# sidiso/surfh

Hardware: AMD Instinct MI355X
Metric: CG-iterations/sec (forward+adjoint) on 251x251x4000 cube (higher is better)
Workload: dtype f32 (storage and accumulation; products as 2-piece fp16 splits -- 3 products per fp32 product, 1 on the far tails of the spectral response -- on the 16-bit matrix cores, in the spectral-blur GEMM and in the DFT passes)

## Files before the change

surfh_amd/csrc/gemm_cc16.hip:

```cpp
#include "gemm_f32.h"
#include "f16_split.h"
#include "lds_attr.h"
#include <cmath>
#include <cstdlib>
#include <type_traits>

typedef float f32x16 __attribute__((ext_vector_type(16)));
typedef _Float16 f16x8 __attribute__((ext_vector_type(8)));
typedef _Float16 f16x4 __attribute__((ext_vector_type(4)));

namespace {

constexpr int BM = 256, BN = 256, BK = 32;
constexpr int ROWS = BM + BN;
constexpr int PIECE = ROWS * BK;
constexpr int STAGE = 2 * PIECE;
constexpr size_t LDS_BYTES = (size_t)2 * STAGE * sizeof(unsigned short);

__global__ __launch_bounds__(256) void split_rows2h_kernel(const float *__restrict__ src, const unsigned *__restrict__ rowmax,
                                                           unsigned short *__restrict__ dst, int ld, long plane) {
    const int row = blockIdx.y;
    const float inv = 1.f / f16x2_scale(__uint_as_float(rowmax[row]));
    const int k4 = (blockIdx.x * 256 + threadIdx.x) * 4;
    if (k4 >= ld) return;
// ... 38 lines not shown

#define CC_MFMA_DRAIN() asm volatile("s_nop 15\n\ts_nop 15\n\ts_nop 7" ::: "memory")

typedef float f32x4v __attribute__((ext_vector_type(4)));

template <int U, int N, bool DMA, bool FAR>
__device__ __forceinline__ void cc16_slot(f32x4v (&acc)[4][8], f16x8 (&A)[4][2], const f16x8 (&Bc)[2][2], f16x8 (&Bn)[2][2], unsigned ran,
                                          unsigned rbn, const char *ka, const char *kb, long pA2, long pB2, const unsigned (&offA)[2],
                                          const unsigned (&offB)[2], unsigned ls) {
    constexpr int i = N / 6, jj = (N / 3) & 1, j = 2 * U + jj, p = N % 3;
    if constexpr (!(CC_EXP & 4) && (!FAR || p == 2))
        asm volatile("v_mfma_f32_16x16x32_f16 %0, %1, %2, %0" : "+v"(acc[i][j]) : "v"(A[i][p == 0 ? 1 : 0]), "v"(Bc[jj][p == 1 ? 1 : 0]));
    if constexpr (N < 4 && !(CC_EXP & 2)) {
        constexpr int jn = 2 * ((U + 1) & 3) + (N >> 1), q = N & 1;
        if constexpr (!FAR || q == 0)
            asm volatile("ds_read_b128 %0, %1 offset:%2" : "=v"(Bn[N >> 1][q]) : "v"(rbn), "n"(q * PIECE * 2 + jn * 16 * BK * 2));
    }
    if constexpr (U == 3 && N % 6 == 5 && !(CC_EXP & 2)) {
        asm volatile("ds_read_b128 %0, %1 offset:%2" : "=v"(A[i][0]) : "v"(ran), "n"(i * 16 * BK * 2));
        if constexpr (!FAR) asm volatile("ds_read_b128 %0, %1 offset:%2" : "=v"(A[i][1]) : "v"(ran), "n"(PIECE * 2 + i * 16 * BK * 2));
    }
    constexpr int d = (U == 3 && N % 3 != 2 && N < 12) ? N - N / 3 : -1;
    if constexpr (DMA && d >= 0 && !(CC_EXP & 1) && (!FAR || d < 4)) {
        constexpr int q = d >> 2, i2 = (d >> 1) & 1;
        if constexpr (d & 1) cc2_dma(kb + q * pB2, offB[i2], ls + (unsigned)((q * PIECE + (BM + i2 * 128) * BK) * 2));
        else cc2_dma(ka + q * pA2, offA[i2], ls + (unsigned)((q * PIECE + i2 * 128 * BK) * 2));
    }
}
template <int U, bool DMA, bool FAR, int N = 0>
__device__ __forceinline__ void cc16_unit(f32x4v (&acc)[4][8], f16x8 (&A)[4][2], const f16x8 (&Bc)[2][2], f16x8 (&Bn)[2][2], unsigned ran,
                                          unsigned rbn, const char *ka, const char *kb, long pA2, long pB2, const unsigned (&offA)[2],
                                          const unsigned (&offB)[2], unsigned ls) {
    if constexpr (N < 24) {
        if constexpr (U == 0 && N == 18 && !(CC_EXP & 2)) {
            if constexpr (FAR) asm volatile("s_waitcnt lgkmcnt(3)" : "+v"(A[3][0]), "+v"(A[3][1]));
            else asm volatile("s_waitcnt lgkmcnt(5)" : "+v"(A[3][0]), "+v"(A[3][1]));
        }
        cc16_slot<U, N, DMA, FAR>(acc, A, Bc, Bn, ran, rbn, ka, kb, pA2, pB2, offA, offB, ls);
        cc16_unit<U, DMA, FAR, N + 1>(acc, A, Bc, Bn, ran, rbn, ka, kb, pA2, pB2, offA, offB, ls);
    }
}
#define CC16_WAITB(n_, B_)                                                                                              \
    asm volatile("s_waitcnt lgkmcnt(" #n_ ")" : "+v"(B_[0][0]), "+v"(B_[1][0]), "+v"(B_[0][1]), "+v"(B_[1][1]))

constexpr int CC2_MAXLIST = 2048;
constexpr size_t LDS3_BYTES = LDS2_BYTES + (size_t)CC2_MAXLIST * sizeof(int);

struct GemmGroup {
    GemmArgs g[GEMM_GROUP_MAX];
    long first[GEMM_GROUP_MAX + 1];
    int n;
};

__global__ __launch_bounds__(512, 1) void gemm_nt_f16x2_cc_kernel(GemmGroup grp) {
    extern __shared__ __attribute__((aligned(16))) unsigned short lds[];
    const long gtotal = grp.first[grp.n], per = (gtotal + 7) / 8;
    const long vg = (long)(blockIdx.x & 7) * per + (blockIdx.x >> 3);
    if ((long)(blockIdx.x >> 3) >= per || vg >= gtotal) return;
    int gi = 0;
    while (gi + 1 < grp.n && vg >= grp.first[gi + 1]) ++gi;
    const long v = vg - grp.first[gi];
    const GemmArgs g = grp.g[gi];
    unsigned char *sctab = reinterpret_cast<unsigned char *>(lds + 2 * STAGE);
    int *klds = reinterpret_cast<int *>(sctab + CC2_MAXSEG * BM);
    const int tid = threadIdx.x, lane = tid & 63, wave = __builtin_amdgcn_readfirstlane(tid >> 6);
    const int Q = g.permP ? BN / g.permP : BN, tilesL = g.permP ? g.permLin / Q : 0, ncol = g.permP ? g.N / g.permLin : 0;
    const int tilesM = (g.M + BM - 1) / BM, tilesN = g.permP ? (ncol + g.permP - 1) / g.permP * tilesL : (g.N + BN - 1) / BN, tiles = tilesM * tilesN;
    auto bcol = [&](int tn_, int v) __attribute__((always_inline)) {
        if (!g.permP) { const int n = tn_ * BN + v; return n < g.N ? n : -1; }
        const int c = (tn_ / tilesL) * g.permP + v / Q;
        return c < ncol ? c * g.permLin + (tn_ % tilesL) * Q + v % Q : -1;
    };
    const int t = (int)(v % tiles), z = (int)(v / tiles);
    const int tm = t % tilesM, tn = t / tilesM;
    const int b = z / g.splitK, sk = z % g.splitK;
    const int m0 = tm * BM;
    const float *bs = g.bscale;

    int nnear, nfar, seg0 = 0, nseg = 0;
    if (g.klist) {
        const int *kl = g.klist + (long)tn * g.klistStride;
        const int NN = kl[0], NF = kl[1];
        const int a0 = (int)((long)NN * sk / g.splitK), a1 = (int)((long)NN * (sk + 1) / g.splitK);
        const int f0 = (int)((long)NF * sk / g.splitK), f1 = (int)((long)NF * (sk + 1) / g.splitK);
        nnear = __builtin_amdgcn_readfirstlane(a1 - a0);
        nfar = __builtin_amdgcn_readfirstlane(f1 - f0);
        for (int e = tid; e < nnear; e += 512) klds[e] = kl[2 + a0 + e];
        for (int e = tid; e < nfar; e += 512) klds[nnear + e] = kl[2 + NN + f0 + e];
        if (bs) nseg = (g.K / g.segLinP) * g.segChunks;
    } else {
        const int Kper = g.K / g.splitK, kbeg = sk * Kper;
        nnear = Kper / BK;
        nfar = 0;
        if (bs) {
            seg0 = cc2_seg_of(kbeg, g.segLinP, g.segChunks);
            nseg = cc2_seg_of(kbeg + Kper - 1, g.segLinP, g.segChunks) - seg0 + 1;
        }
        for (int e = tid; e < nnear; e += 512) {
            const int k = kbeg + e * BK;
            klds[e] = (k / BK) | (bs ? ((k / g.segLinP) * g.segChunks + (k % g.segLinP) / 1024) << 16 : 0);
        }
    }
    for (int e = tid; e < nseg * BM; e += 512) {
        int row = m0 + (e & (BM - 1));
        row = row < g.M ? row : g.M - 1;
        sctab[e] = (unsigned char)(__float_as_uint(bs[(long)(seg0 + (e >> 8)) * g.M + row]) >> 23);
    }

    unsigned offA[2], offB[2];
    {
        const int chunk = (lane & 3) ^ ((-(lane >> 4)) & 3);
#pragma unroll
        for (int i = 0; i < 2; ++i) {
            int m = m0 + (wave + 8 * i) * 16 + (lane >> 2);
            m = m < g.M ? m : g.M - 1;
            offA[i] = (unsigned)(((long)m * g.lda + 8 * chunk) * 2);
            int n = bcol(tn, (wave + 8 * i) * 16 + (lane >> 2));
            n = n >= 0 ? n : g.N - 1;
            offB[i] = (unsigned)(((long)n * g.ldb + 8 * chunk) * 2);
        }
    }
    const char *baseA = cc2_uniform(reinterpret_cast<const char *>(g.A3 + (long)b * g.sA));
    const char *baseB = cc2_uniform(reinterpret_cast<const char *>(g.B16 + (long)b * g.sB));
    const long pA2 = g.pA3 * 2, pB2 = g.pB16 * 2;
    const unsigned ldsw = (unsigned)(size_t)lds + (unsigned)(wave * 16 * BK * 2);
    const unsigned kaddr = (unsigned)(size_t)klds;
    const int l15 = lane & 15, kc = lane >> 4;
    const int wm = wave >> 1, wn = wave & 1;
    f32x4v acc[4][8];
#pragma unroll
    for (int i = 0; i < 4; ++i)
#pragma unroll
        for (int j = 0; j < 8; ++j) acc[i][j] = f32x4v{0.f, 0.f, 0.f, 0.f};
    const unsigned ra0 = (unsigned)(size_t)lds + (unsigned)(((wm * 64 + l15) * BK + ((kc ^ ((-(l15 >> 2)) & 3)) * 8)) * 2);
    const unsigned fbd = (unsigned)((BM + wn * 128 - wm * 64) * BK * 2);
    const bool active = m0 + wm * 64 < g.M;
    const int srow = wm * 64 + 4 * kc;
    int seg = -1;

    f16x8 A[4][2], Bx[2][2], By[2][2];
#define CC_RD(dst_, addr_, off_) asm volatile("ds_read_b128 %0, %1 offset:%2" : "=v"(dst_) : "v"(addr_), "n"(off_))
#define CC_DMA(FAR_, ks_, st_)                                                                                         \
    {                                                                                                                  \
        const char *ka = baseA + (long)(ks_) * (BK * 2), *kb = baseB + (long)(ks_) * (BK * 2);                         \
        const unsigned ls = ldsw + stofs((FAR_), (st_));                                                               \
        _Pragma("unroll") for (int q = 0; q < ((FAR_) ? 1 : 2); ++q) {                                                 \
            _Pragma("unroll") for (int i = 0; i < 2; ++i) {                                                            \
                cc2_dma(ka + q * pA2, offA[i], ls + (q * PIECE + i * 128 * BK) * 2);                                   \
                cc2_dma(kb + q * pB2, offB[i], ls + (q * PIECE + (BM + i * 128) * BK) * 2);                            \
            }                                                                                                          \
        }                                                                                                              \
    }
    auto stofs = [](bool far, int s) __attribute__((always_inline)) {
        return far ? (unsigned)((s >> 1) * (STAGE * 2) + (s & 1) * (PIECE * 2)) : (unsigned)(s * (STAGE * 2));
    };
    __syncthreads();

    auto kloop = [&](auto far_tag, const int lb, const int n) __attribute__((always_inline)) {
        constexpr bool FAR = decltype(far_tag)::value;
        constexpr int D = FAR ? 4 : 2;
        if (n <= 0) return;
        int e[D];
#pragma unroll
        for (int s = 0; s < D; ++s) {
            e[s] = __builtin_amdgcn_readfirstlane(klds[lb + (s < n ? s : n - 1)]);
            CC_DMA(FAR, e[s] & 0xFFFF, s);
        }
        if (FAR) asm volatile("s_waitcnt vmcnt(12)" ::: "memory");
        else asm volatile("s_waitcnt vmcnt(8)" ::: "memory");
        __syncthreads();
        if (!active) {
            for (int kt = 0; kt < n; ++kt) {
                if (FAR) asm volatile("s_waitcnt vmcnt(8)\n\ts_barrier" ::: "memory");
                else asm volatile("s_waitcnt vmcnt(0)\n\ts_barrier" ::: "memory");
                const int ed = __builtin_amdgcn_readfirstlane(klds[lb + (kt + D < n ? kt + D : n - 1)]);
                CC_DMA(FAR, ed & 0xFFFF, kt & (D - 1));
            }
            asm volatile("s_waitcnt vmcnt(0)" ::: "memory");
            return;
        }
        unsigned ra = ra0, rb = ra0 + fbd;
        if (!(CC_EXP & 2)) {
#pragma unroll
            for (int i = 0; i < 4; ++i) {
                CC_RD(A[i][0], ra, 0 + 0);
                if (!FAR) CC_RD(A[i][1], ra, PIECE * 2);
                ra += 16 * BK * 2;
            }
            ra -= 4 * 16 * BK * 2;
            CC_RD(Bx[0][0], rb, 0); CC_RD(Bx[1][0], rb, 16 * BK * 2);
            if (!FAR) { CC_RD(Bx[0][1], rb, PIECE * 2); CC_RD(Bx[1][1], rb, PIECE * 2 + 16 * BK * 2); }
            asm volatile("s_waitcnt lgkmcnt(0)" : "+v"(A[0][0]), "+v"(A[0][1]), "+v"(A[1][0]), "+v"(A[1][1]), "+v"(A[2][0]), "+v"(A[2][1]), "+v"(A[3][0]),
                         "+v"(A[3][1]), "+v"(Bx[0][0]), "+v"(Bx[1][0]), "+v"(Bx[0][1]), "+v"(Bx[1][1]));
        }
        for (int kt = 0; kt < n; ++kt) {
            const int nseg_ = e[0] >> 16;
            if (bs && nseg_ != seg) {
                if (seg >= 0) {
                    const unsigned char *to = sctab + (seg - seg0) * BM + srow, *tn_ = sctab + (nseg_ - seg0) * BM + srow;
                    unsigned so[4], sn[4];
                    bool same = true;
#pragma unroll
                    for (int i = 0; i < 4; ++i) {
                        so[i] = *reinterpret_cast<const unsigned *>(to + i * 16);
                        sn[i] = *reinterpret_cast<const unsigned *>(tn_ + i * 16);
                        same = same && so[i] == sn[i];
                    }
                    if (__builtin_amdgcn_ballot_w64(!same) != 0ull) {
                        CC_MFMA_DRAIN();
#pragma unroll
                        for (int i = 0; i < 4; ++i) {
                            const f32x4v rt = {cc2_pow2_ratio(so[i] & 255u, sn[i] & 255u), cc2_pow2_ratio((so[i] >> 8) & 255u, (sn[i] >> 8) & 255u),
                                               cc2_pow2_ratio((so[i] >> 16) & 255u, (sn[i] >> 16) & 255u), cc2_pow2_ratio(so[i] >> 24, sn[i] >> 24)};
#pragma unroll
                            for (int j = 0; j < 8; ++j) acc[i][j] *= rt;
                            __builtin_amdgcn_sched_barrier(0);
                        }
                    }
                }
                seg = nseg_;
            }
            unsigned ev;
            asm volatile("ds_read_b32 %0, %1" : "=v"(ev) : "v"(kaddr + 4u * (unsigned)(lb + (kt + D < n ? kt + D : n - 1))));
            const char *kz = baseA;
            const unsigned ls2 = ldsw + stofs(FAR, kt & (D - 1));
            cc16_unit<0, false, FAR>(acc, A, Bx, By, ra, rb, kz, kz, pA2, pB2, offA, offB, ls2);
            asm volatile("s_waitcnt lgkmcnt(0)" : "+v"(By[0][0]), "+v"(By[1][0]), "+v"(By[0][1]), "+v"(By[1][1]), "+v"(ev));
            const int en = __builtin_amdgcn_readfirstlane((int)ev);
            const char *ka2 = baseA + (long)(en & 0xFFFF) * (BK * 2), *kb2 = baseB + (long)(en & 0xFFFF) * (BK * 2);
            cc16_unit<1, false, FAR>(acc, A, By, Bx, ra, rb, kz, kz, pA2, pB2, offA, offB, ls2);
            CC16_WAITB(0, Bx);
            cc16_unit<2, false, FAR>(acc, A, Bx, By, ra, rb, kz, kz, pA2, pB2, offA, offB, ls2);
            CC16_WAITB(0, By);
            if (FAR) asm volatile("s_waitcnt vmcnt(8)\n\ts_barrier" ::: "memory");
            else asm volatile("s_waitcnt vmcnt(0)\n\ts_barrier" ::: "memory");
            {
                const unsigned nx = stofs(FAR, (kt + 1) & (D - 1));
                ra = ra0 + nx; rb = ra0 + fbd + nx;
            }
            cc16_unit<3, true, FAR>(acc, A, By, Bx, ra, rb, ka2, kb2, pA2, pB2, offA, offB, ls2);
            if (FAR) { CC16_WAITB(1, Bx); }
            else { CC16_WAITB(2, Bx); }
#pragma unroll
            for (int s = 0; s + 1 < D; ++s) e[s] = e[s + 1];
            e[D - 1] = en;
        }
        asm volatile("s_waitcnt vmcnt(0) lgkmcnt(0)" ::: "memory");
    };
    kloop(std::false_type{}, 0, nnear);
    if (nfar > 0) {
        __syncthreads();
        kloop(std::true_type{}, nnear, nfar);
    }
    if (!active) return;
    CC_MFMA_DRAIN();
#undef CC_DMA
#undef CC_RD
    {
        char *Cb = reinterpret_cast<char *>(g.C + (long)b * g.sC + (long)sk * g.sCsplit + (long)m0 * g.ldc);
        int cj[8];
#pragma unroll
        for (int j = 0; j < 8; ++j) {
            const int c0 = bcol(tn, wn * 128 + j * 16);
            cj[j] = c0 >= 0 ? c0 + l15 : -1;
        }
        const unsigned ldc4 = (unsigned)(g.ldc * 4);
#pragma unroll
        for (int i = 0; i < 4; ++i) {
            float rsc[4];
#pragma unroll
            for (int r = 0; r < 4; ++r) {
                const int lr = srow + i * 16 + r;
                int row = m0 + lr;
                row = row < g.M ? row : g.M - 1;
                rsc[r] = bs ? (seg >= 0 ? __uint_as_float((unsigned)sctab[(seg - seg0) * BM + lr] << 23) : 1.f) : f16x2_scale(__uint_as_float(g.amax[(long)b * g.M + row]));
            }
#pragma unroll
            for (int r = 0; r < 4; ++r) {
                const int row = m0 + srow + i * 16 + r;
                const float sc = rsc[r] * g.sB16;
                const unsigned o_ = (unsigned)(srow + i * 16 + r) * ldc4;
#pragma unroll
                for (int j = 0; j < 8; ++j)
                    if (row < g.M && cj[j] >= 0 && cj[j] < g.N) *reinterpret_cast<float *>(Cb + (o_ + (unsigned)cj[j] * 4u)) = acc[i][j][r] * sc;
            }
        }
    }
}
#undef CC16_WAITB

__global__ __launch_bounds__(256) void split2h_kernel(const float *__restrict__ src, unsigned short *__restrict__ dst, long n4, long plane,
                                                      float inv) {
    const long stride = (long)gridDim.x * 256;
    for (long i = (long)blockIdx.x * 256 + threadIdx.x; i < n4; i += stride) {
        const float4 v = reinterpret_cast<const float4 *>(src)[i];
        const float x0 = v.x * inv, x1 = v.y * inv, x2 = v.z * inv, x3 = v.w * inv;
        const _Float16 h0 = (_Float16)x0, h1 = (_Float16)x1, h2 = (_Float16)x2, h3 = (_Float16)x3;
        f16x4 h = {h0, h1, h2, h3};
        f16x4 l = {(_Float16)(x0 - (float)h0), (_Float16)(x1 - (float)h1), (_Float16)(x2 - (float)h2), (_Float16)(x3 - (float)h3)};
        *reinterpret_cast<f16x4 *>(dst + 4 * i) = h;
        *reinterpret_cast<f16x4 *>(dst + plane + 4 * i) = l;
    }
}

}

float gemm_f16x2_scale(float amax) {
    if (!(amax > 0.f)) return 1.f;
    int e = 0;
    std::frexp(amax, &e);
    int s = (e - 1) - 13;
    s = s < -126 ? -126 : (s > 127 ? 127 : s);
    return std::ldexp(1.f, s);
}

int launch_split2h(hipStream_t stream, const float *src, unsigned short *dst2, long n, long plane, float scale) {
    if (n % 4 || plane % 4 || !(scale > 0.f)) return (int)hipErrorInvalidValue;
    const long n4 = n / 4;
    long nb = (n4 + 255) / 256;
    hipLaunchKernelGGL(split2h_kernel, dim3((unsigned)(nb > 4096 ? 4096 : (nb < 1 ? 1 : nb))), dim3(256), 0, stream, src, dst2, n4, plane,
                       1.f / scale);
    return (int)hipGetLastError();
}

int launch_split_rows2h(hipStream_t stream, const float *src, const unsigned *rowmax, unsigned short *dst2, int rows, int ld, long plane) {
    if (ld % 4 || plane % 4 || rows < 1) return (int)hipErrorInvalidValue;
    hipLaunchKernelGGL(split_rows2h_kernel, dim3((ld / 4 + 255) / 256, rows), dim3(256), 0, stream, src, rowmax, dst2, ld, plane);
    return (int)hipGetLastError();
}

static int check_gemm_nt_f16x2_cc(const GemmArgs &g, long *items) {
    if (g.M % 64 || g.N % 128 || g.K % (BK * g.splitK) || g.splitK < 1 || g.batch < 1 || g.accumulate || g.lda % 8 || g.ldb % 8 || !g.A3 ||
        !g.B16 || g.pA3 % 8 || g.pB16 % 8 || (!g.amax && !g.bscale) || !(g.sB16 > 0.f))
        return (int)hipErrorInvalidValue;
    if (g.bscale && (g.batch != 1 || g.segLinP < BK || g.segLinP % BK || g.segChunks != (g.segLinP + 1023) / 1024 || g.K % g.segLinP))
        return (int)hipErrorInvalidValue;
    if ((double)(BM + 1) * (double)g.ldc * 4.0 >= 2147483648.0) return (int)hipErrorInvalidValue;
    if ((double)g.M * (double)g.lda * 2.0 >= 4294967296.0 || (double)g.N * (double)g.ldb * 2.0 >= 4294967296.0) return (int)hipErrorInvalidValue;
    if (g.klist) {
        if (g.batch != 1 || g.klistStride < 2 + g.K / BK || g.K / BK > CC2_MAXLIST || g.K / BK > 0xFFFF) return (int)hipErrorInvalidValue;
        if (g.bscale && (g.K / g.segLinP) * g.segChunks > CC2_MAXSEG) return (int)hipErrorInvalidValue;
    } else {
        const int Kper = g.K / g.splitK;
        if (Kper / BK > CC2_MAXLIST || g.K / BK > 0xFFFF) return (int)hipErrorInvalidValue;
        if (g.bscale) {
            auto seg_of = [&](int k) { return (k / g.segLinP) * g.segChunks + (k % g.segLinP) / 1024; };
            for (int sk = 0; sk < g.splitK; ++sk)
                if (seg_of(sk * Kper + Kper - 1) - seg_of(sk * Kper) + 1 > CC2_MAXSEG) return (int)hipErrorInvalidValue;
        }
    }
    long tilesN = (g.N + BN - 1) / BN;
    if (g.permP) {
        if ((g.permP != 1 && g.permP != 2 && g.permP != 4 && g.permP != 8) || g.permLin < 1 || g.permLin % (BN / g.permP) || g.N % g.permLin)
            return (int)hipErrorInvalidValue;
        tilesN = (long)((g.N / g.permLin + g.permP - 1) / g.permP) * (g.permLin / (BN / g.permP));
    }
    *items = (long)((g.M + BM - 1) / BM) * tilesN * g.batch * g.splitK;
    return 0;
}

int launch_gemm_nt_f16x2_cc_group(hipStream_t stream, const GemmArgs *gs, int n) {
    if (n < 1 || n > GEMM_GROUP_MAX) return (int)hipErrorInvalidValue;
    GemmGroup grp;
    grp.n = n;
    grp.first[0] = 0;
    for (int i = 0; i < n; ++i) {
        long items = 0;
        if (int e = check_gemm_nt_f16x2_cc(gs[i], &items)) return e;
        grp.g[i] = gs[i];
        grp.first[i + 1] = grp.first[i] + items;
    }
    for (int i = n; i < GEMM_GROUP_MAX; ++i) grp.first[i + 1] = grp.first[n];
    const long total = grp.first[n];
    if (total >= 2147483647L - 8) return (int)hipErrorInvalidValue;
    dim3 grid((unsigned)(8 * ((total + 7) / 8)));
    static unsigned long long attr_done = 0;
    if (int e = ensure_dynamic_lds(gemm_nt_f16x2_cc_kernel, LDS3_BYTES, attr_done)) return e;
    hipLaunchKernelGGL(gemm_nt_f16x2_cc_kernel, grid, dim3(512), LDS3_BYTES, stream, grp);
    return (int)hipGetLastError();
}

int launch_gemm_nt_f16x2_cc(hipStream_t stream, const GemmArgs &g) { return launch_gemm_nt_f16x2_cc_group(stream, &g, 1); }
```

surfh_amd/csrc/gemm_f32.h:

```cpp
#pragma once
#include <hip/hip_runtime.h>
#include <stdint.h>

struct GemmArgs {
    const float *A0 = nullptr, *A1 = nullptr;
    int ksplitA = 1 << 30;
    long lda = 0, sA = 0;
    const float *B0 = nullptr, *B1 = nullptr;
    int ksplitB = 1 << 30;
    long ldb = 0, sB = 0;
    float *C = nullptr;
    long ldc = 0, sC = 0;
    int M = 0, N = 0, K = 0;
    int batch = 1;
    int splitK = 1;
    long sCsplit = 0;
    int accumulate = 0;
    const unsigned short *A3 = nullptr, *B16 = nullptr;
    long pA3 = 0, pB16 = 0;
    float sB16 = 0.f;
    const unsigned *amax = nullptr;
    const float *bscale = nullptr;
    int segLinP = 0, segChunks = 0;
    const int *klist = nullptr;
    int klistStride = 0;
    int permP = 0, permLin = 0;
};

int launch_gemm_f32(hipStream_t stream, const GemmArgs &g);
int launch_gemm_f64acc(hipStream_t stream, const GemmArgs &g);

int launch_split2h(hipStream_t stream, const float *src, unsigned short *dst2, long n, long plane, float scale);
float gemm_f16x2_scale(float amax);
int launch_gemm_nt_f16x2_cc(hipStream_t stream, const GemmArgs &g);
constexpr int GEMM_GROUP_MAX = 4;
int launch_gemm_nt_f16x2_cc_group(hipStream_t stream, const GemmArgs *g, int n);
int launch_split_rows2h(hipStream_t stream, const float *src, const unsigned *rowmax, unsigned short *dst2, int rows, int ld, long plane);
```

surfh_amd/csrc/plan.hip:

```cpp
#include "plan_internal.h"

#include <atomic>

namespace surfh_impl {

namespace {
thread_local std::string g_err;
}

int fail(const char *fmt, ...) {
    char buf[1024];
    va_list ap;
    va_start(ap, fmt);
    vsnprintf(buf, sizeof buf, fmt, ap);
    va_end(ap);
    g_err = buf;
    return 1;
}

namespace {
std::atomic<int64_t> g_alloc_live{0}, g_alloc_total{0}, g_alloc_fail_at{0};
}
int dev_raw_alloc(void **p, size_t bytes) {
    *p = nullptr;
// ... 655 lines not shown
    const Route r0 = decide_route(rin, OTF_NONE);
    const bool ilv = r0.interleaved();
    {
        const int nkb = p->Nb / 2 + 1;
        const size_t nsp = (size_t)2 * p->PL * LP;
        if (p->sotf.zeros(nsp)) return bail(1);
        std::vector<float> row((size_t)2 * p->KBP * LP);
        for (int a = 0; a < p->Na; ++a) {
            std::fill(row.begin(), row.end(), 0.f);
            for (int l = 0; l < p->Lown; ++l) {
                if (p->planes[l] < 0) continue;
                const double *src = cfg->sotf ? cfg->sotf + ((size_t)p->planes[l] * p->Na + a) * nkb * 2 : nullptr;
                for (int k = 0; k < nkb; ++k) {
                    const float vr = src ? (float)src[2 * k] : 1.f, vi = src ? (float)src[2 * k + 1] : 0.f;
                    if (ilv) {
                        row[((size_t)k * LP + l) * 2] = vr;
                        row[((size_t)k * LP + l) * 2 + 1] = vi;
                    } else {
                        row[(size_t)k * LP + l] = vr;
                        row[((size_t)p->KBP + k) * LP + l] = vi;
                    }
                }
            }
            if (ilv) {
                if (hipMemcpy(p->sotf + (size_t)a * p->KBP * LP * 2, row.data(), (size_t)2 * p->KBP * LP * sizeof(float),
                              hipMemcpyHostToDevice) != hipSuccess)
                    return bail(fail("sotf upload failed"));
            } else
            for (int c = 0; c < 2; ++c)
                if (hipMemcpy(p->sotf + ((size_t)c * p->PL + (size_t)a * p->KBP) * LP, row.data() + (size_t)c * p->KBP * LP,
                              (size_t)p->KBP * LP * sizeof(float), hipMemcpyHostToDevice) != hipSuccess)
                    return bail(fail("sotf upload failed"));
        }
    }
    if (p->T > 0) {
        std::vector<float> t((size_t)p->T * LP, 0.f);
        for (int k = 0; k < p->T; ++k)
            for (int l = 0; l < p->Lown; ++l)
                if (p->planes[l] >= 0) t[(size_t)k * LP + l] = (float)cfg->templates[(size_t)k * p->Lc + p->planes[l]];
        if (p->tpl.upload(t)) return bail(1);
        p->tpl_host.assign(cfg->templates, cfg->templates + (size_t)p->T * p->Lc);
    }
    {
        std::vector<float> Fi, Gi, Gf, Ff, GiT, GfT;
        build_dft(p, Fi, Gi, Gf, Ff, GiT, GfT);
        if (p->Fi.upload(Fi) || p->Gi.upload(Gi) || p->Gf.upload(Gf) || p->Ff.upload(Ff) || p->GiT.upload(GiT) || p->GfT.upload(GfT)) return bail(1);
    }
    {
        p->wblur_fp32 = env_on("SURFH_WBLUR_FP32", false);
        p->overlap = env_on("SURFH_OVERLAP", false);
        if (p->overlap && hipStreamCreateWithFlags(&p->stream2, hipStreamNonBlocking) != hipSuccess) return bail(fail("hipStreamCreate failed"));
        p->gather_grouped = env_on("SURFH_GATHER_GROUPED", true);
        p->gemm_grouped = env_on("SURFH_GEMM_GROUPED", true);
        p->scatter_grouped = env_on("SURFH_SCATTER_GROUPED", true);
        p->gather_sorted = env_on("SURFH_GATHER_SORTED", true);
        const int ha = p->Na / 2 + 1, hb = p->Nb / 2 + 1;
        p->MPa = (ha + 127) / 128 * 128; p->KPa = (ha + 15) / 16 * 16;
        p->MPb = (hb + 127) / 128 * 128; p->KPb = (hb + 15) / 16 * 16;
        if (p->KPa > p->NAP || p->KPb > p->NBP || p->KPb > p->KBP) return bail(fail("cube too small for the folded DFT"));
        const double sa = 1.0 / std::sqrt((double)p->Na), sb = 1.0 / std::sqrt((double)p->Nb);
        std::vector<float> Cma((size_t)p->MPa * p->KPa, 0.f), Sma(Cma.size(), 0.f);
        for (int r = 0; r < ha; ++r)
            for (int k = 0; k < ha; ++k) {
                const double th = 2.0 * M_PI * (double)(((long)r * k) % p->Na) / (double)p->Na;
                Cma[(size_t)r * p->KPa + k] = (float)(std::cos(th) * sa);
                Sma[(size_t)r * p->KPa + k] = (float)(std::sin(th) * sa);
            }
        std::vector<float> Gc((size_t)p->MPb * p->KPb, 0.f), Gs(Gc.size(), 0.f), Cf(Gc.size(), 0.f), Sf(Gc.size(), 0.f);
        for (int b = 0; b < hb; ++b)
            for (int k = 0; k < hb; ++k) {
                const double th = 2.0 * M_PI * (double)(((long)b * k) % p->Nb) / (double)p->Nb;
                const double w = (k == 0 || (p->Nb % 2 == 0 && k == p->Nb / 2)) ? 1.0 : 2.0;
                Gc[(size_t)b * p->KPb + k] = (float)(w * std::cos(th) * sb);
                Gs[(size_t)b * p->KPb + k] = (float)(w * std::sin(th) * sb);
                Cf[(size_t)k * p->KPb + b] = (float)(std::cos(th) * sb);
                Sf[(size_t)k * p->KPb + b] = (float)(std::sin(th) * sb);
            }
        if (p->Cma.upload(Cma) || p->Sma.upload(Sma) || p->Gc.upload(Gc) || p->Gs.upload(Gs) || p->Cf.upload(Cf) || p->Sf.upload(Sf)) return bail(1);
        if (cfg->verify) {
            p->verify = true;
            p->wblur_fp32 = true;
            p->overlap = false;
        }
        if (r0.ax_a == AX_H2 || r0.ax_b == AX_H2) {
            if ((r0.ax_a == AX_H2 && p->MPa != 128) || (r0.ax_b == AX_H2 && p->MPb != 128)) return bail(fail("internal: dft_h2 needs 128-row folded matrices"));
            std::vector<unsigned short> im(3 * DFT_H2_IMAGE_HALFS, 0);
            if (r0.ax_a == AX_H2) p->h2kA[0] = dft_h2_build_image(Cma.data(), Sma.data(), p->MPa, p->KPa, p->KPa, im.data());
            if (r0.ax_b == AX_H2) {
                p->h2kA[1] = dft_h2_build_image(Gc.data(), Gs.data(), p->MPb, p->KPb, p->KPb, im.data() + DFT_H2_IMAGE_HALFS);
                p->h2kA[2] = dft_h2_build_image(Cf.data(), Sf.data(), p->MPb, p->KPb, p->KPb, im.data() + 2 * DFT_H2_IMAGE_HALFS);
            }
            if (p->h2img.upload(im)) return bail(1);
        }
        if (r0.ax_a == AX_CT && dft_ct_plan_create(p->Na, &p->ctA)) return bail(fail("dft_ct plan (n_alpha = %d) failed", p->Na));
        if (r0.ax_b == AX_CT) {
            if (r0.ax_a == AX_CT && p->Nb == p->Na) p->ctB = &p->ctA;
            else if (dft_ct_plan_create(p->Nb, &p->ctB_own)) return bail(fail("dft_ct plan (n_beta = %d) failed", p->Nb));
        }
        OtfSupport found;
        if (otf_support(p, cfg, r0, rin.on(SW_OTF_RANGES), &found)) return bail(1);
        p->route = decide_route(rin, found);
        if (p->route.fused_tail) {
            const size_t npart = dft_h2_adjmix_part_floats(p->LP, p->Nb / 2 + 1, p->otf_nvalid);
            if (!npart) return bail(fail("the fused adjoint tail could not size its partial sums"));
            if (p->adjmix_part.alloc(npart)) return bail(1);
        }
// ... 249 lines not shown
```

surfh_amd/csrc/plan_diag.hip:

```cpp
#include "plan_internal.h"
#include "mm_step.h"

extern "C" {

int surfh_profile_enable(surfh_plan *p, int32_t on) {
    if (!p) return fail("null plan");
    p->prof = on != 0;
    return 0;
}
int surfh_profile_filter(surfh_plan *p, const char *prefix) {
    if (!p) return fail("null plan");
    p->prof_filter = prefix ? prefix : "";
    return 0;
}
int32_t surfh_profile_count(surfh_plan *p) {
    if (!p) return -1;
    hipSetDevice(p->dev);
    prof_collect(p);
    return (int32_t)p->acc_names.size();
}
int surfh_profile_get(surfh_plan *p, int32_t i, const char **name, int64_t *launches, double *ms) {
    if (!p || i < 0 || i >= (int32_t)p->acc_names.size()) return fail("bad profile index");
    auto &e = p->acc[p->acc_names[i]];
    *name = p->acc_names[i].c_str();
// ... 157 lines not shown
    if (!step) return fail("null argument");
    mm_step2(dBd, dBm, mBm, dg, mg, &step[0], &step[1]);
    return 0;
}

static long g_selftest_ksteps[2] = {0, 0};
int surfh_gemm_selftest_ksteps(int64_t near_far[2]) {
    near_far[0] = g_selftest_ksteps[0]; near_far[1] = g_selftest_ksteps[1];
    return 0;
}

static double g_selftest_ms = -1.0;
int surfh_gemm_selftest_ms(double *ms) {
    if (!ms) return fail("null argument");
    *ms = g_selftest_ms;
    return 0;
}

int surfh_gemm_selftest(int32_t device, int32_t M, int32_t N, int32_t K, int32_t split_k, const float *A,
                        const float *B, float *C) {
    HIP_OK(hipSetDevice(device));
    DevBuf<float> dA, dB, dC;
    const int sk = std::max(1, (int)split_k);
    if (dA.alloc((size_t)M * K) || dB.alloc((size_t)K * N) || dC.alloc((size_t)sk * M * N)) return 1;
    HIP_OK(hipMemcpy(dA, A, (size_t)M * K * 4, hipMemcpyHostToDevice));
    HIP_OK(hipMemcpy(dB, B, (size_t)K * N * 4, hipMemcpyHostToDevice));
    GemmArgs g;
    g.A0 = dA; g.lda = K; g.B0 = dB; g.ldb = N; g.C = dC; g.ldc = N;
    g.M = M; g.N = N; g.K = K; g.splitK = sk; g.sCsplit = (long)M * N;
    int rc;
    const char *mode = getenv("SURFH_SELFTEST_F16X2");
    if (mode && (mode[0] == '1' || mode[0] == '2')) {
        std::vector<float> bt((size_t)N * K);
        for (int k = 0; k < K; ++k)
            for (int n = 0; n < N; ++n) bt[(size_t)n * K + k] = B[(size_t)k * N + n];
        HIP_OK(hipMemcpy(dB, bt.data(), bt.size() * 4, hipMemcpyHostToDevice));
        g.ldb = K;
        DevBuf<unsigned short> dB16, dA16;
        DevBuf<unsigned> dmax;
        float amB = 0.f;
        for (float v : bt) amB = std::max(amB, std::fabs(v));
        std::vector<unsigned> rows((size_t)M, 0u);
        for (int m = 0; m < M; ++m) {
            float am = 0.f;
            for (int k = 0; k < K; ++k) am = std::max(am, std::fabs(A[(size_t)m * K + k]));
            memcpy(&rows[m], &am, 4);
        }
        if (dB16.alloc(bt.size() * 2) || dmax.alloc(rows.size()) || dA16.alloc((size_t)M * K * 2)) return 1;
        HIP_OK(hipMemcpy(dmax, rows.data(), rows.size() * sizeof(unsigned), hipMemcpyHostToDevice));
        g.sB16 = gemm_f16x2_scale(amB); g.B16 = dB16; g.pB16 = (long)bt.size(); g.amax = dmax;
        rc = launch_split2h(nullptr, dB, dB16, (long)bt.size(), (long)bt.size(), g.sB16);
        if (rc == 0) rc = launch_split_rows2h(nullptr, dA, dmax, dA16, M, K, (long)M * K);
        g.A3 = dA16; g.pA3 = (long)M * K;
        DevBuf<int> dkl;
        g_selftest_ksteps[0] = g_selftest_ksteps[1] = 0;
        if (mode[0] == '2') {
            std::vector<int> kl;
            const char *ep = getenv("SURFH_SELFTEST_PERM");
            const int lin = ep ? atoi(ep) : 0;
            if (lin > 0) { g.permP = 4; g.permLin = lin; }
            build_klist(bt.data(), N, K, K, 0, 0, 1.0 / 256, 1.0 / 1024, &kl, &g.klistStride, &g_selftest_ksteps[0], &g_selftest_ksteps[1], g.permP,
                        g.permLin);
            if (dkl.upload(kl)) return 1;
            g.klist = dkl;
        }
        if (rc == 0) rc = launch_gemm_nt_f16x2_cc(nullptr, g);
        if (rc == 0) rc = (int)hipDeviceSynchronize();
        g_selftest_ms = -1.0;
        const char *er = getenv("SURFH_SELFTEST_REPEAT");
        const int nrep = er ? atoi(er) : 0;
        if (rc == 0 && nrep > 0) {
            hipEvent_t ea, eb;
            HIP_OK(hipEventCreate(&ea));
            HIP_OK(hipEventCreate(&eb));
            for (int i = 0; i < 3 && rc == 0; ++i) rc = launch_gemm_nt_f16x2_cc(nullptr, g);
            hipEventRecord(ea, nullptr);
            for (int i = 0; i < nrep && rc == 0; ++i) rc = launch_gemm_nt_f16x2_cc(nullptr, g);
            hipEventRecord(eb, nullptr);
            if (rc == 0) rc = (int)hipEventSynchronize(eb);
            float ms = 0.f;
            if (rc == 0) rc = (int)hipEventElapsedTime(&ms, ea, eb);
            if (rc == 0) g_selftest_ms = (double)ms / nrep;
            hipEventDestroy(ea);
            hipEventDestroy(eb);
        }
    } else {
        rc = launch_gemm_f32(nullptr, g);
    }
    if (rc == 0) rc = (int)hipDeviceSynchronize();
    std::vector<float> h((size_t)sk * M * N);
    if (rc == 0) rc = (int)hipMemcpy(h.data(), dC, h.size() * 4, hipMemcpyDeviceToHost);
    if (rc) return fail("gemm selftest failed: %s", hipGetErrorString((hipError_t)rc));
    for (size_t i = 0; i < (size_t)M * N; ++i) {
        float s = 0.f;
        for (int k = 0; k < sk; ++k) s += h[(size_t)k * M * N + i];
        C[i] = s;
    }
    return 0;
}

}
```

surfh_amd/csrc/plan_internal.h:

```cpp
#pragma once

#include <hip/hip_runtime.h>

#include <algorithm>
#include <array>
#include <cfloat>
#include <cmath>
#include <cstdarg>
#include <cstdio>
#include <cstdlib>
#include <cstring>
#include <functional>
#include <map>
#include <string>
#include <vector>

#include "../../include/surfh_amd.h"
#include "dev_buf.h"
#include "dft_h2.h"
#include "dft_ct.h"
#include "gemm_f32.h"
#include "kernels.h"
#include "tplgrad.h"

// ... 97 lines not shown
inline void route_fields(const Route &r, int64_t f[8]) {
    const int64_t v[8] = {r.ax_a, r.ax_b, r.mix, r.prod, r.fused_tail, r.support, r.tpl_spectral, r.spec_calls};
    std::copy(v, v + 8, f);
}

}

using namespace surfh_impl;

struct PlanHandles {
    int dev = 0;
    hipStream_t stream = nullptr;
    bool own_stream = false;
    hipStream_t stream2 = nullptr;
    std::vector<hipEvent_t> sync_ev;
    std::vector<ProfRec> pending;
    std::vector<hipEvent_t> pool;
    PlanHandles() = default;
    PlanHandles(const PlanHandles &) = delete;
    PlanHandles &operator=(const PlanHandles &) = delete;
    ~PlanHandles() {
        for (auto &r : pending) {
            hipEventDestroy(r.a);
            hipEventDestroy(r.b);
        }
        for (hipEvent_t e : pool) hipEventDestroy(e);
        for (hipEvent_t e : sync_ev) hipEventDestroy(e);
        if (stream2) hipStreamDestroy(stream2);
        if (own_stream && stream) hipStreamDestroy(stream);
    }
};

struct surfh_plan : PlanHandles {
    bool overlap = false;
    size_t sync_next = 0;
    int Na = 0, Nb = 0, Lc = 0, T = 0, NAP = 0, NBP = 0, KAP = 0, KBP = 0;
    long PL = 0, PLc = 0;
    int lo = 0, hi = 0, Lown = 0, LP = 0;
    int Leff = 0;
    struct Seg { int start, len, coff; };
    std::vector<Seg> segs;
    std::vector<int> planes;
    int compact(int l) const {
        for (auto &g : segs) if (l >= g.start && l <= g.start + g.len) return g.coff + (l - g.start);
        return -1;
    }
    DevBuf<float> sotf, tpl, mhat, spec, ycol, cube, maps_pad, ycol_maps;
    DevBuf<float> Fi, Gi, Gf, Ff, GiT, GfT;
    DevBuf<float> Cma, Sma, Gc, Gs, Cf, Sf;
    int MPa = 0, KPa = 0, MPb = 0, KPb = 0;
    int n_cu = 256;
    bool gather_sorted = true;
    bool gemm_grouped = true;
    bool scatter_grouped = true;
    bool gather_grouped = true;
    bool wblur_fp32 = false;
    bool verify = false;
    int prior_kind = 0;
    int pot[3] = {0, 0, 0};
    int coupling = 0;
    Route route;
    DevBuf<unsigned short> h2img;
    DftCtPlan ctA, ctB_own;
    const DftCtPlan *ctB = &ctB_own;
    int a_lo = 0, a_hi = 0, b_lo = 0, b_hi = 0;
    DevBuf<float> ycol_adj;
    DevBuf<float> adjmix_part;
    DevBuf<int> otf_vlist, otf_kbstart;
    int otf_nvalid = 0;
    DevBuf<int> otf_tabs;
    DevBuf<float> ycol_mix;
    int h2kA[3] = {0, 0, 0};
    DevBuf<float> io_x, io_y, io_cube, hth, mhat2;
    DevBuf<float> gcube;
    std::vector<Channel> ch;
    long isize = 0, osize = 0;
    DevBuf<float> dw, dwy;
    int im_F = 0, im_d = 0;
    long im_osize = 0;
    DevBuf<float> im_g, im_xpad, im_xhat, im_zpad, im_zhat, im_io;
    DevBuf<float> im_y, im_w, im_wy;
    double im_mu = 0.0;
    int ycm_planes = 0;
    std::vector<double> tpl_host;
    DevBuf<int> tg_cidx, tg_pidx;
    DevBuf<double> tg_part;
    DevBuf<float> tg_keep, tg_v[6];
    bool tg_mhat_ready = false;
    DevBuf<float> cg_x, cg_r, cg_d, cg_q, cg_b, cg_y, cg_qm, cg_dd;
    DevBuf<float> cg_hg;
    DevBuf<float> cpl_w;
    DevBuf<float> rb_y, rb_u, rb_ag, rb_am;
    DevBuf<double> dscal, dscratch;
    DevBuf<float> po_y, po_eps, po_er, po_ec, po_eta, po_xhat;
    DevBuf<double> po_S;
    DevBuf<float> nn_z;
    float *nn_u = nullptr, *nn_w = nullptr;
    DevBuf<float> nn_rho;
    DevBuf<double> nn_part;
    double *nn_sums = nullptr;
    DevBuf<double> cg_hist;
    int cg_hist_n = 0;
    DevBuf<double> pl_sc;
    DevBuf<double> pl_hsc;
    DevBuf<double> pl_hpar;
    float *pl_x = nullptr;
// ... 90 lines not shown
```

surfh_amd/csrc/plan_ops.hip:

```cpp
#include "plan_internal.h"

namespace surfh_impl {

int prior_add(surfh_plan *p, hipStream_t st, const float *d, float *q, int n_img, float mu_reg) {
    return p->prior_kind == 1 ? launch_prior_joint_add(st, d, q, n_img, p->Na, p->Nb, mu_reg) : launch_prior_add(st, d, q, n_img, p->Na, p->Nb, mu_reg);
}

namespace {

int gemm32(surfh_plan *p, hipStream_t st, const GemmArgs &g) { return p->verify ? launch_gemm_f64acc(st, g) : launch_gemm_f32(st, g); }

int rfft2_planes(surfh_plan *p, const float *src, float *dst, int B) {
    GemmArgs g;
    g.A0 = src; g.lda = p->NBP; g.sA = p->PLc;
    g.B0 = p->Gf; g.ldb = 2 * p->KBP; g.sB = 0;
    g.C = p->ycol_maps; g.ldc = 2 * p->KBP; g.sC = (long)p->NAP * 2 * p->KBP;
    g.M = p->NAP; g.N = 2 * p->KBP; g.K = p->NBP; g.batch = B;
    {
        Prof pr(p, "gemm_dft_rows_fwd_maps");
        LAUNCH_OK(gemm32(p, p->stream, g));
    }
    GemmArgs h;
    h.A0 = p->Ff; h.lda = 2 * p->NAP; h.sA = 0;
    h.B0 = p->ycol_maps; h.B1 = p->ycol_maps + p->KBP; h.ksplitB = p->NAP; h.ldb = 2 * p->KBP;
// ... 338 lines not shown
    }
    IrfftCall inv;
    if (p->route.mix) {
        inv.mix = call.head == OpCall::H_SPECTRA ? call.spectra_in : p->mhat;
        inv.alpha_range_only = hand_over;
        if (irfft2_cube(p, p->sotf, p->cube, inv)) return 1;
    } else if (p->route.prod) {
        ProdOperand po;
        po.prod = p->sotf;
        inv.prod = &po;
        if (irfft2_cube(p, p->mhat, p->cube, inv)) return 1;
    } else {
        {
            Prof pr(p, "specmix_fwd");
            LAUNCH_OK(launch_specmix_fwd(s, p->mhat, p->sotf, p->tpl, p->spec, p->T, p->PL, p->LP, p->route.interleaved()));
        }
        if (irfft2_cube(p, p->spec, p->cube)) return 1;
    }
    hipStream_t sB = (p->overlap && p->stream2) ? p->stream2 : s;
    for (auto &c : p->ch) {
        const bool f16 = c.W16 != nullptr;
        {
            Prof pr(p, "spmm_gather_fwd");
            if (c.Xs16 && c.fwd.g.NG)
                LAUNCH_OK(launch_spmm_group_gather_f16(s, c.fwd.g, p->cube, c.Xs16, (long)c.NP * c.K, c.nlam, c.bscale, c.NP, c.K, c.LinP));
            else if (c.Xs16)
                LAUNCH_OK(launch_spmm_rows_f16(s, c.fwd.t, p->cube, c.Xs16, (long)c.NP * c.K, c.nlam, c.bscale, c.NP, c.K, c.LinP));
            else if (p->verify)
                LAUNCH_OK(launch_spmm_rows_f64acc(s, c.fwd.t, p->cube, c.Xs, c.nlam, 0));
            else
                LAUNCH_OK(launch_spmm_rows(s, c.fwd.t, p->cube, c.Xs, c.nlam, 0));
        }
        if (c.bsum) {
            Prof pr(p, "y_transpose");
            LAUNCH_OK(launch_cube_from_lam_inner(s, c.Xs + c.shift, y + c.yoff, 0, c.Lin, 1, c.P * c.S * c.aout, 1, c.LinP));
            continue;
        }
        if (chain(p, s, sB)) return 1;
        GemmArgs g;
        g.A0 = c.Xs; g.lda = c.K;
        g.C = c.Cpart; g.ldc = c.LdetP;
        g.M = c.NP; g.N = c.LdetP; g.K = c.K; g.splitK = c.splitK; g.sCsplit = (long)c.NP * c.LdetP;
        {
            Prof pr(p, "gemm_wblur_fwd", sB);
            if (p->wblur_fp32) {
                g.B0 = c.Wt; g.ldb = c.LdetP;
                LAUNCH_OK(gemm32(p, sB, g));
            } else {
                g.ldb = c.K;
                g.B16 = c.W16; g.pB16 = (long)c.LdetP * c.K; g.sB16 = c.sW;
                g.A3 = c.Xs16; g.pA3 = (long)c.NP * c.K;
                g.bscale = c.bscale; g.segLinP = c.LinP; g.segChunks = (c.LinP + 1023) / 1024;
                g.klist = c.klF; g.klistStride = c.klFs;
                LAUNCH_OK(launch_gemm_nt_f16x2_cc(sB, g));
            }
        }
        if (hand_over && c.ymat16 && c.wmat) {
            Prof pr(p, "ymat16w_from_cpart", sB);
            LAUNCH_OK(launch_ymat16w_from_cpart(sB, c.Cpart, (long)c.NP * c.LdetP, c.splitK, c.ymat16, (long)c.NP * c.LdetP, c.amax, c.NP,
                                                c.P * c.S * c.aout, c.Ldet, c.LdetP, c.wmat));
        } else if (hand_over && c.ymat16) {
            Prof pr(p, "ymat16_from_cpart", sB);
            LAUNCH_OK(launch_ymat16_from_cpart(sB, c.Cpart, (long)c.NP * c.LdetP, c.splitK, c.ymat16, (long)c.NP * c.LdetP, c.amax, c.NP,
                                               c.P * c.S * c.aout, c.Ldet, c.LdetP));
        } else {
            Prof pr(p, "y_from_cpart", sB);
            LAUNCH_OK(launch_y_from_cpart(sB, c.Cpart, (long)c.NP * c.LdetP, c.splitK, y + c.yoff, c.P * c.S, c.Ldet,
                                          c.aout, c.LdetP));
        }
    }
    if (chain(p, sB, s)) return 1;
    return 0;
}

int adjoint_dev(surfh_plan *p, const float *y, float *x, const OpCall &call) {
    hipStream_t s = p->stream;
    const bool ref = call.ref, handed_over = call.hand_over;
    hipStream_t sB = (p->overlap && p->stream2) ? p->stream2 : s;
    if (chain(p, s, sB)) return 1;
    float *const acc = (!ref && p->gcube) ? p->gcube : p->cube;
    if (acc == p->cube) {
        Prof pr(p, "fill_zero");
        LAUNCH_OK(launch_fill_zero(s, p->cube, (long)p->NBP * p->NAP * p->LP));
    }
    auto prepare = [&](Channel &c) -> int {
        const bool f16 = c.W16 != nullptr;
        if (handed_over && f16 && c.ymat16) return 0;
        {
            Prof pr(p, "ymat_from_y", sB);
            LAUNCH_OK(launch_ymat_from_y(sB, y + c.yoff, c.ymat, c.P * c.S, c.Ldet, c.aout, c.LdetP, f16 ? c.pmax : nullptr,
                                         f16 ? c.amax : nullptr, c.NP));
        }
        if (f16 && !p->wblur_fp32)
            LAUNCH_OK(launch_split_rows2h(sB, c.ymat, c.amax, c.ymat16, c.NP, c.LdetP, (long)c.NP * c.LdetP));
        return 0;
    };
    auto gemm_args = [&](Channel &c) {
        GemmArgs g;
        g.A0 = c.ymat; g.lda = c.LdetP;
        g.C = c.Xs; g.ldc = c.K;
        g.M = c.NP; g.N = c.K; g.K = c.LdetP;
        if (p->wblur_fp32) {
            g.B0 = c.W; g.ldb = c.K;
        } else if (c.W16) {
            g.K = (c.Ldet + 31) / 32 * 32;
            g.ldb = c.LdetP;
            g.B16 = c.Wt16; g.pB16 = (long)c.LdetP * c.K; g.sB16 = c.sW; g.amax = c.amax;
            g.A3 = c.ymat16; g.pA3 = (long)c.NP * c.LdetP;
            g.klist = c.klA; g.klistStride = c.klAs;
            if (c.klA && c.permA) { g.permP = c.permA; g.permLin = c.LinP; }
        }
        return g;
    };
    auto scatter = [&](Channel &c) -> int {
        Prof pr(p, ref ? "spmm_degrid_ref" : "spmm_scatter_adj");
        if (p->verify)
            LAUNCH_OK(launch_spmm_rows_f64acc(s, ref ? c.adjRef.t : c.adjT.t, c.Xs, acc, c.nlam, 1));
        else if (!ref && c.adjT.g.NG)
            LAUNCH_OK(launch_spmm_group_scatter(s, c.adjT.g, c.Xs, acc, c.nlam));
        else
            LAUNCH_OK(launch_spmm_rows(s, ref ? c.adjRef.t : c.adjT.t, c.Xs, acc, c.nlam, 1));
        return 0;
    };
    std::vector<char> gemm_done(p->ch.size(), 0);
    if (p->gemm_grouped && !p->wblur_fp32 && !p->verify) {
        std::vector<GemmArgs> ga;
        std::vector<size_t> gc;
        for (size_t ci = 0; ci <= p->ch.size(); ++ci) {
            const bool last = ci == p->ch.size();
            if (!last) {
                Channel &c = p->ch[ci];
                if (c.bsum || !c.W16 || (ref && !c.has_ref)) continue;
                if (prepare(c)) return 1;
                ga.push_back(gemm_args(c)); gc.push_back(ci);
            }
            if (!ga.empty() && (last || (int)ga.size() == GEMM_GROUP_MAX)) {
                {
                    Prof pr(p, "gemm_wblur_adj", sB);
                    LAUNCH_OK(launch_gemm_nt_f16x2_cc_group(sB, ga.data(), (int)ga.size()));
                }
                for (size_t i : gc) gemm_done[i] = 1;
                ga.clear(); gc.clear();
            }
        }
    }
    for (size_t ci = 0; ci < p->ch.size(); ++ci) {
        Channel &c = p->ch[ci];
        if (ref && !c.has_ref) return fail("adjoint_ref needs the gridding_t tables (gt_*) in the channel descriptor");
        if (c.bsum) {
            {
                Prof pr(p, "y_transpose");
                LAUNCH_OK(launch_cube_to_lam_inner(s, y + c.yoff, c.Xs + c.shift, 0, c.Lin, 1, c.P * c.S * c.aout, 1, c.LinP));
            }
            if (scatter(c)) return 1;
            continue;
        }
        if (!gemm_done[ci]) {
            if (prepare(c)) return 1;
            const GemmArgs g = gemm_args(c);
            Prof pr(p, "gemm_wblur_adj", sB);
            if (p->wblur_fp32 || !c.W16) LAUNCH_OK(gemm32(p, sB, g));
            else LAUNCH_OK(launch_gemm_nt_f16x2_cc(sB, g));
// ... 709 lines not shown
```

Measured before the change: 352.8.

## Overlap GEMM prologue table fill with first DMA stages and specialize full-tile stores

Adds an EDGES template variant of the fp16x2 cc GEMM kernel. It issues the first k-step DMAs straight from the klist before filling the LDS k-list and scale tables, so the prologue table fill overlaps the initial global loads instead of sitting behind a barrier. It also batches the per-segment scale loads, caches the per-row amax scales in LDS, and uses an unguarded store path for full tiles. The cost is more code complexity and extra LDS use for row scales; the selftest is also changed to pre-initialise C.

Result: no change. 355.2, median of 6 (+0.7%).

```diff
diff --git a/surfh_amd/csrc/gemm_cc16.hip b/surfh_amd/csrc/gemm_cc16.hip
--- a/surfh_amd/csrc/gemm_cc16.hip
+++ b/surfh_amd/csrc/gemm_cc16.hip
@@ -114,6 +114,7 @@
     int n;
 };
 
+template <bool EDGES>
 __global__ __launch_bounds__(512, 1) void gemm_nt_f16x2_cc_kernel(GemmGroup grp) {
     extern __shared__ __attribute__((aligned(16))) unsigned short lds[];
     const long gtotal = grp.first[grp.n], per = (gtotal + 7) / 8;
@@ -140,34 +141,61 @@
     const float *bs = g.bscale;
 
     int nnear, nfar, seg0 = 0, nseg = 0;
+    int NN = 0, a0 = 0, f0 = 0, kbeg = 0;
+    const int *kl = nullptr;
     if (g.klist) {
-        const int *kl = g.klist + (long)tn * g.klistStride;
-        const int NN = kl[0], NF = kl[1];
-        const int a0 = (int)((long)NN * sk / g.splitK), a1 = (int)((long)NN * (sk + 1) / g.splitK);
-        const int f0 = (int)((long)NF * sk / g.splitK), f1 = (int)((long)NF * (sk + 1) / g.splitK);
+        kl = g.klist + (long)tn * g.klistStride;
+        if constexpr (EDGES) kl = reinterpret_cast<const int *>(cc2_uniform(reinterpret_cast<const char *>(kl)));
+        NN = kl[0];
+        const int NF = kl[1];
+        a0 = (int)((long)NN * sk / g.splitK);
+        f0 = (int)((long)NF * sk / g.splitK);
+        const int a1 = (int)((long)NN * (sk + 1) / g.splitK), f1 = (int)((long)NF * (sk + 1) / g.splitK);
         nnear = __builtin_amdgcn_readfirstlane(a1 - a0);
         nfar = __builtin_amdgcn_readfirstlane(f1 - f0);
-        for (int e = tid; e < nnear; e += 512) klds[e] = kl[2 + a0 + e];
-        for (int e = tid; e < nfar; e += 512) klds[nnear + e] = kl[2 + NN + f0 + e];
         if (bs) nseg = (g.K / g.segLinP) * g.segChunks;
     } else {
-        const int Kper = g.K / g.splitK, kbeg = sk * Kper;
+        const int Kper = g.K / g.splitK;
+        kbeg = sk * Kper;
         nnear = Kper / BK;
         nfar = 0;
         if (bs) {
             seg0 = cc2_seg_of(kbeg, g.segLinP, g.segChunks);
             nseg = cc2_seg_of(kbeg + Kper - 1, g.segLinP, g.segChunks) - seg0 + 1;
         }
-        for (int e = tid; e < nnear; e += 512) {
-            const int k = kbeg + e * BK;
-            klds[e] = (k / BK) | (bs ? ((k / g.segLinP) * g.segChunks + (k % g.segLinP) / 1024) << 16 : 0);
-        }
-    }
-    for (int e = tid; e < nseg * BM; e += 512) {
-        int row = m0 + (e & (BM - 1));
-        row = row < g.M ? row : g.M - 1;
-        sctab[e] = (unsigned char)(__float_as_uint(bs[(long)(seg0 + (e >> 8)) * g.M + row]) >> 23);
-    }
+    }
+    auto entry = [&](int i) __attribute__((always_inline)) {
+        if (g.klist) return i < nnear ? kl[2 + a0 + i] : kl[2 + NN + f0 + (i - nnear)];
+        const int k = kbeg + i * BK;
+        return (k / BK) | (bs ? ((k / g.segLinP) * g.segChunks + (k % g.segLinP) / 1024) << 16 : 0);
+    };
+    float *rowsc = reinterpret_cast<float *>(sctab);
+    auto fill_tables = [&]() __attribute__((always_inline)) {
+        for (int e = tid; e < nnear + nfar; e += 512) klds[e] = entry(e);
+        if constexpr (EDGES) {
+            const int lr = tid & (BM - 1), row = m0 + lr < g.M ? m0 + lr : g.M - 1;
+            for (int s0 = tid >> 8; s0 < nseg; s0 += 16) {
+                float v[8];
+#pragma unroll
+                for (int u = 0; u < 8; ++u) v[u] = s0 + 2 * u < nseg ? bs[(long)(seg0 + s0 + 2 * u) * g.M + row] : 0.f;
+#pragma unroll
+                for (int u = 0; u < 8; ++u)
+                    if (s0 + 2 * u < nseg) sctab[(s0 + 2 * u) * BM + lr] = (unsigned char)(__float_as_uint(v[u]) >> 23);
+            }
+        } else {
+            for (int e = tid; e < nseg * BM; e += 512) {
+                int row = m0 + (e & (BM - 1));
+                row = row < g.M ? row : g.M - 1;
+                sctab[e] = (unsigned char)(__float_as_uint(bs[(long)(seg0 + (e >> 8)) * g.M + row]) >> 23);
+            }
+        }
+        if (EDGES && !bs && tid < BM) {
+            const int row = m0 + tid < g.M ? m0 + tid : g.M - 1;
+            rowsc[tid] = f16x2_scale(__uint_as_float(g.amax[(long)b * g.M + row]));
+        }
+    };
+    const bool pre_near = EDGES && nnear > 0, pre_far = EDGES && nnear <= 0 && nfar > 0;
+    if (!pre_near && !pre_far) fill_tables();
 
     unsigned offA[2], offB[2];
     {
@@ -216,18 +244,24 @@
     auto stofs = [](bool far, int s) __attribute__((always_inline)) {
         return far ? (unsigned)((s >> 1) * (STAGE * 2) + (s & 1) * (PIECE * 2)) : (unsigned)(s * (STAGE * 2));
     };
-    __syncthreads();
-
-    auto kloop = [&](auto far_tag, const int lb, const int n) __attribute__((always_inline)) {
+    if (!pre_near && !pre_far) __syncthreads();
+
+    auto kloop = [&](auto far_tag, const int lb, const int n, const bool pre) __attribute__((always_inline)) {
         constexpr bool FAR = decltype(far_tag)::value;
         constexpr int D = FAR ? 4 : 2;
         if (n <= 0) return;
         int e[D];
 #pragma unroll
         for (int s = 0; s < D; ++s) {
-            e[s] = __builtin_amdgcn_readfirstlane(klds[lb + (s < n ? s : n - 1)]);
-            CC_DMA(FAR, e[s] & 0xFFFF, s);
-        }
+            const int idx = lb + (s < n ? s : n - 1);
+            e[s] = __builtin_amdgcn_readfirstlane(EDGES && pre ? entry(idx) : klds[idx]);
+            if constexpr (!EDGES) CC_DMA(FAR, e[s] & 0xFFFF, s);
+        }
+        if constexpr (EDGES) {
+#pragma unroll
+            for (int s = 0; s < D; ++s) CC_DMA(FAR, e[s] & 0xFFFF, s);
+        }
+        if (EDGES && pre) fill_tables();
         if (FAR) asm volatile("s_waitcnt vmcnt(12)" ::: "memory");
         else asm volatile("s_waitcnt vmcnt(8)" ::: "memory");
         __syncthreads();
@@ -309,10 +343,10 @@
         }
         asm volatile("s_waitcnt vmcnt(0) lgkmcnt(0)" ::: "memory");
     };
-    kloop(std::false_type{}, 0, nnear);
+    kloop(std::false_type{}, 0, nnear, pre_near);
     if (nfar > 0) {
         __syncthreads();
-        kloop(std::true_type{}, nnear, nfar);
+        kloop(std::true_type{}, nnear, nfar, pre_far);
     }
     if (!active) return;
     CC_MFMA_DRAIN();
@@ -327,26 +361,34 @@
             cj[j] = c0 >= 0 ? c0 + l15 : -1;
         }
         const unsigned ldc4 = (unsigned)(g.ldc * 4);
-#pragma unroll
-        for (int i = 0; i < 4; ++i) {
-            float rsc[4];
-#pragma unroll
-            for (int r = 0; r < 4; ++r) {
-                const int lr = srow + i * 16 + r;
-                int row = m0 + lr;
-                row = row < g.M ? row : g.M - 1;
-                rsc[r] = bs ? (seg >= 0 ? __uint_as_float((unsigned)sctab[(seg - seg0) * BM + lr] << 23) : 1.f) : f16x2_scale(__uint_as_float(g.amax[(long)b * g.M + row]));
-            }
-#pragma unroll
-            for (int r = 0; r < 4; ++r) {
-                const int row = m0 + srow + i * 16 + r;
-                const float sc = rsc[r] * g.sB16;
-                const unsigned o_ = (unsigned)(srow + i * 16 + r) * ldc4;
-#pragma unroll
-                for (int j = 0; j < 8; ++j)
-                    if (row < g.M && cj[j] >= 0 && cj[j] < g.N) *reinterpret_cast<float *>(Cb + (o_ + (unsigned)cj[j] * 4u)) = acc[i][j][r] * sc;
-            }
-        }
+        const bool full = EDGES && m0 + BM <= g.M && (g.permP ? (tn / tilesL + 1) * g.permP <= ncol : (tn + 1) * BN <= g.N);
+        auto store_tile = [&](auto full_tag) __attribute__((always_inline)) {
+            constexpr bool FULL = decltype(full_tag)::value;
+#pragma unroll
+            for (int i = 0; i < 4; ++i) {
+                float rsc[4];
+#pragma unroll
+                for (int r = 0; r < 4; ++r) {
+                    const int lr = srow + i * 16 + r;
+                    int row = m0 + lr;
+                    row = row < g.M ? row : g.M - 1;
+                    rsc[r] = bs ? (seg >= 0 ? __uint_as_float((unsigned)sctab[(seg - seg0) * BM + lr] << 23) : 1.f)
+                                : (EDGES ? rowsc[lr] : f16x2_scale(__uint_as_float(g.amax[(long)b * g.M + row])));
+                }
+#pragma unroll
+                for (int r = 0; r < 4; ++r) {
+                    const int row = m0 + srow + i * 16 + r;
+                    const float sc = rsc[r] * g.sB16;
+                    const unsigned o_ = (unsigned)(srow + i * 16 + r) * ldc4;
+#pragma unroll
+                    for (int j = 0; j < 8; ++j)
+                        if (FULL || (row < g.M && cj[j] >= 0 && cj[j] < g.N))
+                            *reinterpret_cast<float *>(Cb + (o_ + (unsigned)cj[j] * 4u)) = acc[i][j][r] * sc;
+                }
+            }
+        };
+        if (full) store_tile(std::true_type{});
+        else store_tile(std::false_type{});
     }
 }
 #undef CC16_WAITB
@@ -436,9 +478,14 @@
     const long total = grp.first[n];
     if (total >= 2147483647L - 8) return (int)hipErrorInvalidValue;
     dim3 grid((unsigned)(8 * ((total + 7) / 8)));
-    static unsigned long long attr_done = 0;
-    if (int e = ensure_dynamic_lds(gemm_nt_f16x2_cc_kernel, LDS3_BYTES, attr_done)) return e;
-    hipLaunchKernelGGL(gemm_nt_f16x2_cc_kernel, grid, dim3(512), LDS3_BYTES, stream, grp);
+    static unsigned long long attr_done[2] = {0, 0};
+    if (gs[0].edges) {
+        if (int e = ensure_dynamic_lds(gemm_nt_f16x2_cc_kernel<true>, LDS3_BYTES, attr_done[1])) return e;
+        hipLaunchKernelGGL(gemm_nt_f16x2_cc_kernel<true>, grid, dim3(512), LDS3_BYTES, stream, grp);
+    } else {
+        if (int e = ensure_dynamic_lds(gemm_nt_f16x2_cc_kernel<false>, LDS3_BYTES, attr_done[0])) return e;
+        hipLaunchKernelGGL(gemm_nt_f16x2_cc_kernel<false>, grid, dim3(512), LDS3_BYTES, stream, grp);
+    }
     return (int)hipGetLastError();
 }
 
diff --git a/surfh_amd/csrc/gemm_f32.h b/surfh_amd/csrc/gemm_f32.h
--- a/surfh_amd/csrc/gemm_f32.h
+++ b/surfh_amd/csrc/gemm_f32.h
@@ -25,6 +25,7 @@
     const int *klist = nullptr;
     int klistStride = 0;
     int permP = 0, permLin = 0;
+    bool edges = true;
 };
 
 int launch_gemm_f32(hipStream_t stream, const GemmArgs &g);
diff --git a/surfh_amd/csrc/plan.hip b/surfh_amd/csrc/plan.hip
--- a/surfh_amd/csrc/plan.hip
+++ b/surfh_amd/csrc/plan.hip
@@ -731,6 +731,7 @@
         if (p->overlap && hipStreamCreateWithFlags(&p->stream2, hipStreamNonBlocking) != hipSuccess) return bail(fail("hipStreamCreate failed"));
         p->gather_grouped = env_on("SURFH_GATHER_GROUPED", true);
         p->gemm_grouped = env_on("SURFH_GEMM_GROUPED", true);
+        p->gemm_edges = env_on("SURFH_GEMM_EDGES", true);
         p->scatter_grouped = env_on("SURFH_SCATTER_GROUPED", true);
         p->gather_sorted = env_on("SURFH_GATHER_SORTED", true);
         const int ha = p->Na / 2 + 1, hb = p->Nb / 2 + 1;
diff --git a/surfh_amd/csrc/plan_diag.hip b/surfh_amd/csrc/plan_diag.hip
--- a/surfh_amd/csrc/plan_diag.hip
+++ b/surfh_amd/csrc/plan_diag.hip
@@ -233,6 +233,8 @@
         rc = launch_split2h(nullptr, dB, dB16, (long)bt.size(), (long)bt.size(), g.sB16);
         if (rc == 0) rc = launch_split_rows2h(nullptr, dA, dmax, dA16, M, K, (long)M * K);
         g.A3 = dA16; g.pA3 = (long)M * K;
+        g.edges = env_on("SURFH_GEMM_EDGES", true);
+        for (int s = 0; s < sk; ++s) HIP_OK(hipMemcpy((float *)dC + (size_t)s * M * N, C, (size_t)M * N * 4, hipMemcpyHostToDevice));
         DevBuf<int> dkl;
         g_selftest_ksteps[0] = g_selftest_ksteps[1] = 0;
         if (mode[0] == '2') {
diff --git a/surfh_amd/csrc/plan_internal.h b/surfh_amd/csrc/plan_internal.h
--- a/surfh_amd/csrc/plan_internal.h
+++ b/surfh_amd/csrc/plan_internal.h
@@ -173,6 +173,7 @@
     int n_cu = 256;
     bool gather_sorted = true;
     bool gemm_grouped = true;
+    bool gemm_edges = true;
     bool scatter_grouped = true;
     bool gather_grouped = true;
     bool wblur_fp32 = false;
diff --git a/surfh_amd/csrc/plan_ops.hip b/surfh_amd/csrc/plan_ops.hip
--- a/surfh_amd/csrc/plan_ops.hip
+++ b/surfh_amd/csrc/plan_ops.hip
@@ -414,6 +414,7 @@
                 g.A3 = c.Xs16; g.pA3 = (long)c.NP * c.K;
                 g.bscale = c.bscale; g.segLinP = c.LinP; g.segChunks = (c.LinP + 1023) / 1024;
                 g.klist = c.klF; g.klistStride = c.klFs;
+                g.edges = p->gemm_edges;
                 LAUNCH_OK(launch_gemm_nt_f16x2_cc(sB, g));
             }
         }
@@ -470,6 +471,7 @@
             g.B16 = c.Wt16; g.pB16 = (long)c.LdetP * c.K; g.sB16 = c.sW; g.amax = c.amax;
             g.A3 = c.ymat16; g.pA3 = (long)c.NP * c.LdetP;
             g.klist = c.klA; g.klistStride = c.klAs;
+            g.edges = p->gemm_edges;
             if (c.klA && c.permA) { g.permP = c.permA; g.permLin = c.LinP; }
         }
         return g;
```
